# vedantsawal/Cost-and-Carbon-Aware-Kubernetes-Autoscaler

Measured on AMD Instinct MI355X. Metric: policy-evaluated cluster-steps/sec, higher is better.
Workload: dtype int32+int64+f64; 1 GPU; config2: 1e5 clusters x 1 deployment x 1440 one-minute steps, HPA + peak/off-peak, 16-type catalog; scenarios_per_gpu=100000, steps_per_rollout=1440, mode=trajectory, schedule=lane-skewed (single deployment), trace_layout=wave-tiled [wave][T][lanes] (built by the first rollout), parallelism=scenario-sharded x1

## Files before the change

cost-and-carbon-aware-kubernetes-autoscaler_amd/csrc/rollout_d1.hip:

```cpp
#include <hip/hip_runtime.h>
#include <stdint.h>

#include "../../include/ccka.h"
#include "d1_common.h"
#include "kparams.h"

#pragma clang fp contract(off)

namespace ccka {

namespace {

struct Best {
  double s;
  int k;
  int info;
  int price;
};

__device__ __forceinline__ bool better(double s2, int k2, double s, int k) {
  return s2 < s || (s2 == s && k2 < k);
}

__device__ __forceinline__ void take_if_better(Best& a, const Best& b) {
// ... 13 lines not shown
  Best o;
  const long long b = __double_as_longlong(a.s);
  const int lo = __builtin_amdgcn_readlane((int)(b & 0xffffffffLL), l);
  const int hi = __builtin_amdgcn_readlane((int)(b >> 32), l);
  o.s = __longlong_as_double(((long long)hi << 32) | (unsigned int)lo);
  o.k = __builtin_amdgcn_readlane(a.k, l);
  o.info = __builtin_amdgcn_readlane(a.info, l);
  o.price = __builtin_amdgcn_readlane(a.price, l);
  return o;
}

}

__global__ void __launch_bounds__(256) table_kernel(TableParams q) {
  const int lane = threadIdx.x & (WAVE - 1);
  const int64_t key = ((int64_t)blockIdx.x * blockDim.x + threadIdx.x) / WAVE;
  const int64_t nkeys = (int64_t)q.R * 24 * q.NZI * 3 * q.NW;
  if (key >= nkeys) return;
  int64_t x = key;
  const int wi = (int)(x % q.NW); x /= q.NW;
  const int cmi = (int)(x % 3); x /= 3;
  const int zi = (int)(x % q.NZI); x /= q.NZI;
  const int rh = (int)x;
  const uint32_t cm = (uint32_t)cmi + 1u, zm = q.zmasks[zi];
  const double wc = q.offer ? 0.0 : q.wc1000[wi];
  const double ci = q.ci_gpwh[rh];
  const int32_t* tile = q.price + (int64_t)rh * q.K * q.Z * 2;
  int2* out = q.table + key * q.JT;
  const double INF = __builtin_inf();
  Best cs{INF, 0x7fffffff, -1, 0}, ca{INF, 0x7fffffff, -1, 0};
  int jmax = 0;
  for (int base = 0; base < q.K; base += WAVE) {
    const int pos = base + lane;
    const bool v = pos < q.K;
    const int k = v ? q.order[pos] : 0;
    const int c1 = v ? q.cap1s[pos] : 0;
    const int c1n = pos + 1 < q.K ? q.cap1s[pos + 1] : 0;
    Best bs{INF, 0x7fffffff, -1, 0}, ba{INF, 0x7fffffff, -1, 0};
    if (v) {
      const double carbon = q.types[k].p_ref_w * ci;
      for (int z = 0; z < q.Z; ++z) {
        if (!(zm >> z & 1u)) continue;
        for (int c = 0; c < 2; ++c) {
          if (!(cm & (uint32_t)capbit(c))) continue;
          const int pr = tile[(k * q.Z + z) * 2 + c];
          if (pr <= 0) continue;
          const double score = (double)pr + wc * carbon;
          const int info = k | z << 10 | c << 12;
          if (score < ba.s) { ba.s = score; ba.k = k; ba.info = info; ba.price = pr; }
          if (c == 0 && score < bs.s) { bs.s = score; bs.k = k; bs.info = info; bs.price = pr; }
        }
      }
      if (ba.info >= 0) jmax = max(jmax, c1);
    }
#pragma unroll
    for (int off = 1; off < WAVE; off <<= 1) {
      const Best os = shfl_up_best(bs, off), oa = shfl_up_best(ba, off);
      if (lane >= off) { take_if_better(bs, os); take_if_better(ba, oa); }
    }
    take_if_better(bs, cs);
    take_if_better(ba, ca);
    if (v && c1 > c1n) {
      const Best& w = (!q.offer && bs.info >= 0) ? bs : ba;
      const int info = w.info >= 0 ? (w.info | q.cap1t[w.k] << 16) : -1;
      const int hi = min(c1, q.JT - 1);
      for (int n = c1n + 1; n <= hi; ++n) out[n] = make_int2(w.price, info);
    }
    cs = readlane_best(bs, WAVE - 1);
    ca = readlane_best(ba, WAVE - 1);
  }
#pragma unroll
  for (int o = 32; o > 0; o >>= 1) jmax = max(jmax, __shfl_xor(jmax, o));
  if (lane == 0) {
    q.jtab[key / q.NW] = jmax;
    out[0] = make_int2(0, jmax);
  }
}

namespace {

__device__ __forceinline__ int opqv(int v) {
  asm volatile("" : "+v"(v));
  return v;
}
__device__ __forceinline__ D1Rule opq_rule(const D1Rule& r) {
  D1Rule o;
  o.sel = opq(r.sel);
  o.n = opq(r.n);
  o.stab_mask = opq(r.stab_mask);
  o._pad = 0;
#pragma unroll
  for (int q = 0; q < 2; ++q) {
    o.type[q] = opq(r.type[q]);
    o.value[q] = opq(r.value[q]);
    o.pmask[q] = opq(r.pmask[q]);
    o.factor[q] = opq(r.factor[q]);
  }
#pragma unroll
  for (int w = 0; w < 4; ++w) {
    o.stab16[w] = opq(r.stab16[w]);
    o.pm16[0][w] = opq(r.pm16[0][w]);
    o.pm16[1][w] = opq(r.pm16[1][w]);
  }
  return o;
}

__device__ __forceinline__ int rate_limit1(const D1Rule& R, bool up, int cur, const uint32_t* del) {
  if (R.sel == CCKA_SELECT_DISABLED) return cur;
  const bool min_sel = R.sel == CCKA_SELECT_MIN;
  long long res = (up == min_sel) ? 0x7fffffffLL : -0x80000000LL;
#pragma unroll
  for (int q = 0; q < 2; ++q) {
    if (q >= R.n) break;
    int added = 0, removed = 0;
    if (R.pmask[q]) {
      const short2v z = {0, 0};
#pragma unroll
      for (int w = 0; w < 4; ++w) {
        const short2v d = as_s2(del[w]), m = as_s2((uint32_t)R.pm16[q][w]);
        added = __builtin_amdgcn_sdot2(__builtin_elementwise_max(d, z), m, added, false);
        removed = __builtin_amdgcn_sdot2(__builtin_elementwise_max(z - d, z), m, removed, false);
      }
    }
    const long long pst = (long long)cur - added + removed;
    long long pr;
    if (R.type[q] == CCKA_HPA_PODS) pr = up ? pst + R.value[q] : pst - R.value[q];
    else if (up) pr = (int)ceil((double)pst * R.factor[q]);
    else pr = (int)((double)pst * R.factor[q]);
    res = (up == min_sel) ? min(res, pr) : max(res, pr);
  }
  return (int)res;
}

}

#define D1_STAMP(k)                                          \
  if constexpr (STAMPS) {                                    \
    __builtin_amdgcn_sched_barrier(0);                       \
    const uint64_t now_ = __builtin_amdgcn_s_memtime();      \
    __builtin_amdgcn_sched_barrier(0);                       \
    st_acc[k] += now_ - st_last;                             \
    st_last = now_;                                          \
  }

constexpr int D1_RB = 64;
constexpr int D1_K = 2;
constexpr int D1_VMN = 4;
constexpr int D1_S = 8;
constexpr int D1_BACK = CCKA_HIST;
static_assert(D1_VMN + 4 * D1_S + D1_BACK <= D1_RB && D1_RB - D1_S - D1_BACK - D1_VMN >= 2 * D1_S,
              "ring too small for the DMA lead");
constexpr int D1_RING_BYTES = D1_RB * WAVE * 4;
constexpr int D1_PRIO_HI = 3;
__device__ __forceinline__ void d1_dma_row(const int32_t* src, uint32_t lds_row) {
  unsigned keep;
  asm volatile(
      "s_mov_b32 %0, m0\n\t"
      "s_mov_b32 m0, %2\n\t"
      "s_nop 0\n\t"
      "global_load_lds_dword %1, off\n\t"
      "s_mov_b32 m0, %0"
      : "=&s"(keep)
      : "v"(src), "s"(lds_row)
      : "memory");
}
__device__ __forceinline__ void d1_wait_rows() { asm volatile("s_waitcnt vmcnt(%0)" ::"n"(D1_VMN) : "memory"); }
__device__ __forceinline__ void d1_wait_all() { asm volatile("s_waitcnt vmcnt(0)" ::: "memory"); }

__device__ __forceinline__ uint32_t xcd_block(uint32_t b, uint32_t n) {
  const uint32_t x = b & 7u, k = b >> 3, q = n >> 3, r = n & 7u;
  return x * q + min(x, r) + k;
}

template <int MAXN, int MAXP, bool STAMPS, int OCC, bool BDEF, bool DRIFT = false, int NSUB = 1, int HE = 8,
          bool G3 = false, bool KEDA = false>
__global__ void __launch_bounds__(256, OCC) rollout_d1_kernel(D1Params p) {
  static_assert(NSUB == 1 || (NSUB == 4 && BDEF), "15 s sync: lean default path");
  static_assert(!KEDA || (BDEF && NSUB == 1 && !DRIFT), "KEDA: default behavior, one decision per step");
  static_assert(HE == 8 || (HE == 4 && NSUB == 1 && BDEF), "4-record ring: default behavior, one decision per step");
  static_assert(!G3 || (DRIFT && MAXP == 2), "G3: the DRIFT instantiation, two pools");
  constexpr int HW = NSUB == 1 ? HE / 2 : 10;
  constexpr int JR = NSUB == 1 ? HE : 5;
  uint64_t st_acc[12] = {0, 0, 0, 0, 0, 0, 0, 0, 0, 0, 0, 0};
  uint64_t st_last = STAMPS ? __builtin_amdgcn_s_memtime() : 0;
  extern __shared__ __attribute__((aligned(16))) int4 s_acc[];
  for (int x = threadIdx.x; x < p.K; x += blockDim.x) {
    const long long idle = p.acc[x * 3 + 0];
    s_acc[x] = make_int4((int)(idle & 0xffffffffLL), (int)(idle >> 32), (int)p.acc[x * 3 + 1], (int)p.acc[x * 3 + 2]);
  }
  const bool ldt = p.lds_tab;
  const uint32_t tab_off = ((uint32_t)p.K * 16u + 255u) / 256u * 256u + (blockDim.x / WAVE) * (uint32_t)D1_RING_BYTES;
  const int n_pr = p.R * 24 * p.K * p.Z * 2;
  const int n_pr8 = (n_pr + 1) & ~1;
  int* const s_price = reinterpret_cast<int*>(reinterpret_cast<char*>(s_acc) + tab_off);
  double* const s_ci = reinterpret_cast<double*>(s_price + n_pr8);
  int* const s_jtab = reinterpret_cast<int*>(s_ci + p.R * 24);
  if (ldt) {
    for (int x = threadIdx.x; x < n_pr; x += blockDim.x) s_price[x] = p.price[x];
    for (int x = threadIdx.x; x < p.R * 24; x += blockDim.x) s_ci[x] = p.ci_gpwmin[x];
    for (int x = threadIdx.x; x < p.R * 24 * p.NZI * 3; x += blockDim.x) s_jtab[x] = p.jtab[x];
  }
  __syncthreads();
  const int lane = threadIdx.x & (WAVE - 1);
  const int64_t wv = (int64_t)xcd_block(blockIdx.x, gridDim.x) * (blockDim.x / WAVE) + (threadIdx.x / WAVE);
  const int64_t i = wv * p.lpw + lane;
  if (lane >= p.lpw || i >= p.N) return;

  const int r = p.region ? (int)p.region[i] : 0;
  const int target = KEDA ? 1 : (p.target ? (int)p.target[i] : p.target0);
  const int mx = KEDA ? opq(p.k_max) : (p.maxr ? (int)p.maxr[i] : p.maxr0);
  const int dwin = (!KEDA && p.down_stab) ? (int)p.down_stab[i] : p.dstab0;
  const int nd = min(NSUB == 1 ? __popc(window_mask(dwin)) : (dwin > 15 ? (dwin - 1) / 15 : 0), 2 * HW);
  const int dnmask = NSUB == 1 ? window_mask(dwin) : 0;
  const int reset_ca = p.reset_ca ? (int)p.reset_ca[i] : p.reset_ca0;
  const int pswitch = p.pswitch ? (int)p.pswitch[i] : p.pswitch0;
  const int wi = p.wci ? (int)p.wci[i] : 0;
  const uint32_t capsel = p.cap_sel ? (uint32_t)p.cap_sel[i] : (uint32_t)p.capsel0;
  const int minr = KEDA ? max(opq(p.k_min), 1) : opq(p.minr), req = opq(p.req_cpu), limit = opq(p.limit);
  const int kthr = KEDA ? opq(p.k_thr) : 1, kact = KEDA ? opq(p.k_act) : 0, kcds = KEDA ? opq(p.k_cds) : 0;
  const bool kmin0 = KEDA && opq(p.k_min) == 0;
  const float rkthr = __builtin_amdgcn_rcpf((float)kthr);
  int ulo = max(0, (int)floor(p.tol_lo * (double)target) - 2);
  while ((double)ulo / (double)target < p.tol_lo) ++ulo;
  int uhi = (int)floor(p.tol_hi * (double)target) + 2;
  while ((double)uhi / (double)target > p.tol_hi) --uhi;
  const float rtarget = __builtin_amdgcn_rcpf((float)target);

  const int NP = opq(p.NP), NZI = opq(p.NZI), NW = opq(p.NW), JT = opq(p.JT);
  const int maxn = opq(p.maxn), ablate = CCKA_ABLATE_BUILD ? opq(p.ablate) : 0, pdb_member = opq(p.pdb_member);
  const int pdb_pct = opq(p.pdb_pct), slo_util = opq(p.slo_util), delay = opq(p.delay);
  const int base_nodes = opq(p.base_nodes), base_type = opq(p.base_type);
  const int K = opq(p.K), Z = opq(p.Z), T = opq(p.T);
  const int ps = opq(p.peak_start) % 1440, pe = opq(p.peak_end) % 1440;
  const int ps_raw = opq(p.peak_start), pe_raw = opq(p.peak_end);
  const int sm0 = opq(p.start_minute) % 1440;
  const long long base_nw = opq(p.base_nw);
  const GLOBAL_AS int32_t* const price = opq_ptr(p.price);
  const GLOBAL_AS double* const ci_gpwmin = opq_ptr(p.ci_gpwmin);
  const GLOBAL_AS int2* const table = opq_ptr(p.table);
  const GLOBAL_AS int2* const table2 = opq_ptr(p.table2);
  const int drift_on = opq(p.drift_on), replace = opq(p.replace), multi = G3 ? opq(p.multi) : 0;
  const GLOBAL_AS int32_t* const jtab = opq_ptr(p.jtab);
  GLOBAL_AS int4* const traj = opq_ptr(reinterpret_cast<int4*>(p.traj));
  const D1Rule rup = [&] { if constexpr (BDEF) return d1_default_rule(true); else return opq_rule(p.up); }();
  const D1Rule rdn = [&] { if constexpr (BDEF) return d1_default_rule(false); else return opq_rule(p.dn); }();
  int budget[MAXP];
#pragma unroll
  for (int q = 0; q < MAXP; ++q) budget[q] = opq(p.budget[q]);

  int ppol[MAXP], pcas[MAXP], pzi[MAXP], pJ[MAXP];
  uint32_t pcm[MAXP], pmask[MAXP];
#pragma unroll
  for (int q = 0; q < MAXP; ++q) {
    ppol[q] = 0; pcas[q] = 0; pzi[q] = -1; pcm[q] = 0; pJ[q] = 0; pmask[q] = 0;
    if (q < NP) {
#pragma unroll
      for (int s = 0; s < 2; ++s) {
        const D1Patch& x = p.patch[q][s];
        if (x.policy) ppol[q] = x.policy;
        if (x.cas >= 0) pcas[q] = s == 1 ? (reset_ca + CCKA_STEP_SECONDS - 1) / CCKA_STEP_SECONDS : x.cas;
        if (x.zi >= 0) pzi[q] = x.zi;
        if (x.cm) pcm[q] = (uint32_t)x.cm;
      }
    }
  }

  auto cas_of = [&](uint32_t info) {
    const int m1 = -(int)(info >> 13 & 1u), m2 = -(int)(info >> 14 & 1u);
    const int lo = pcas[0] ^ ((pcas[0] ^ pcas[MAXP > 1 ? 1 : 0]) & m1);
    if constexpr (MAXP <= 2) {
      return lo;
    } else {
      const int hi = pcas[2] ^ ((pcas[2] ^ pcas[3]) & m1);
      return lo ^ ((lo ^ hi) & m2);
    }
  };
  auto casc = [](int c) { return min(c, 0xFFFF); };

  uint32_t sinfo[MAXN];
  int sready[MAXN], slc[MAXN], scas[MAXN], spods[MAXN], sprice[MAXN], scap[MAXN];
  uint32_t sdyn[MAXN];
  int salloc[MAXN];
  int sallocr[MAXN];
#pragma unroll
  for (int n = 0; n < MAXN; ++n) {
    sinfo[n] = 0; sready[n] = 0; slc[n] = 0; scas[n] = 0; spods[n] = 0; sprice[n] = 0; scap[n] = 0;
    sdyn[n] = 0; salloc[n] = 0; sallocr[n] = 0;
  }
  uint32_t used = 0, rdy = 0, cmask = 0;
  auto dyn_of = [&](int n) -> uint32_t {
    if constexpr (G3) return (uint32_t)s_acc[sinfo[n] & 1023u].z;
    else return sdyn[n];
  };
  auto alloc_of = [&](int n) -> int {
    if constexpr (G3) return s_acc[sinfo[n] & 1023u].w;
    else return salloc[n];
  };
  constexpr bool kAllocR = NSUB == 1 && !G3;
  auto alloc_ready = [&](int n) -> uint32_t {
    if constexpr (kAllocR) return (uint32_t)sallocr[n];
    else return (rdy >> n & 1u) ? (uint32_t)alloc_of(n) : 0u;
  };
  auto cas_slot = [&](int n) -> int {
    if constexpr (G3) return casc(cas_of(sinfo[n]));
    else return scas[n];
  };
  uint32_t dmask = 0, srcm = 0, repm = 0;
  auto taint = [&]() -> uint32_t { return DRIFT ? (srcm | repm) : 0u; };
  auto od_slots = [&]() {
    uint32_t m = 0;
#pragma unroll
    for (int n = MAXN - 1; n >= 0; --n) m = 2 * m + (sinfo[n] >> 12 & 1u);
    return m & used;
  };
  const uint32_t slot_mask = maxn >= 32 ? 0xFFFFFFFFu : ((1u << maxn) - 1u);

  int replicas = p.replicas0, placed = 0, rpods = 0;
  uint32_t hdn[HW], hup[4], hdel[4] = {0, 0, 0, 0};
  uint32_t dn16[HW];
#pragma unroll
  for (int w = 0; w < 4; ++w) hup[w] = 0x7FFF7FFFu;
#pragma unroll
  for (int w = 0; w < HW; ++w) {
    hdn[w] = 0x80008000u;
    dn16[w] = (2 * w < nd ? 0xFFFFu : 0u) | (2 * w + 1 < nd ? 0xFFFF0000u : 0u);
  }
  int next_ready = 0x7fffffff, nsp = 0, nod = 0;
  int kcd = kcds, q_klo = 0, q_khi = -1, kb_cur = -1;
  bool q_kcd = false;
  bool k_act_step = false;
  auto keda_band = [&](int cur) {
    if (!KEDA || cur == kb_cur) return;
    kb_cur = cur;
    if (cur <= 0) { q_klo = 0; q_khi = -1; return; }
    const double D = (double)kthr * (double)cur;
// ... 60 lines not shown
    const int rc = min(max(cur, upr), dnr);
    int lo = minr, hi = mx;
    if constexpr (BDEF) {
      hi = rc > cur ? min(hi, max(2 * cur, cur + 4)) : hi;
      lo = rc < cur ? max(lo, 0) : lo;
    } else {
      if (proposal != cur) {
        if (rc > cur) hi = min(hi, max(rate_limit1(rup, true, cur, hdel), cur));
        else if (rc < cur) lo = max(lo, min(rate_limit1(rdn, false, cur, hdel), cur));
      }
    }
    return rc < lo ? lo : (rc > hi ? hi : rc);
  };
  auto hpa_eval = [&](int L, int cur, int ready, float rbd, float rbc) -> HpaOut {
    HpaOut o;
    const bool metric = cur <= mx && cur >= minr && ready > 0 && !(cur == 0 && minr != 0);
    int util = 0, proposal = cur;
    {
      const int rcapv = ready * limit;
      const int usage = (limit > 0 && rcapv < L) ? rcapv : L;
      const int a = usage * 100;
      const int dreq = ready * req;
      const int dcur = cur * req;
      bool slow = usage < 0 || usage > 21474836;
      util = fdiv_nb(a, dreq, rbd, slow);
      int nu = 0;
      if (cur > ready) nu = fdiv_nb(a, dcur, rbc, slow);
      if (__builtin_expect(metric && slow, 0))
        util = (int)(((long long)usage * 100) / ((long long)ready * req));
      const bool unready_up = cur > ready && util > target;
      int u = util, base = ready;
      if (unready_up) { u = nu; base = cur; }
      if (__builtin_expect(metric && slow && unready_up, 0))
        u = (int)(((long long)usage * 100) / ((long long)cur * req));
      const bool keep = (u >= ulo && u <= uhi) || (unready_up && u < target);
      bool slow2 = (uint32_t)u > 0xFFFFu;
      const int x = u * base;
      const int q = fdiv_nb(x, target, rtarget, slow2);
      const bool exactm = x == q * target;
      int c = q + (exactm ? 0 : 1);
      if (__builtin_expect(metric && !keep && (exactm || slow2), 0))
        c = (int)ceil(((double)u / (double)target) * (double)base);
      const int pe2 = unready_up ? max(cur, c) : c;
      proposal = (metric && !keep) ? pe2 : cur;
    }
    o.util = util;
    o.proposal = proposal;
    o.ran = metric;
    o.hpa_path = !(cur == 0 && minr != 0);
    int desired = cur > mx ? mx : (cur < minr && o.hpa_path ? minr : cur);
    if (metric && !ablated(ablate, 8)) desired = behave(proposal, cur);
    o.desired = desired;
    return o;
  };
  auto keda_eval = [&](int L, int cur, int ts) -> HpaOut {
    HpaOut o{};
    const bool act = L > kact;
    const bool cool = !act && kmin0 && ts >= kcd;
    if (act) kcd = ts + kcds;
    k_act_step = act;
    o.util = 0;
    o.proposal = cur;
    o.ran = false;
    o.hpa_path = false;
    int desired = cur;
    if (cur == 0) {
      desired = act ? 1 : 0;
    } else if (cool) {
      desired = 0;
    } else {
      o.hpa_path = true;
      if (cur > mx) {
        desired = mx;
      } else if (cur < minr) {
        desired = minr;
      } else {
        int prop = cur;
        if (L < q_klo || L > q_khi) {
          bool slow = L < 0;
          const int q = fdiv_nb(max(L, 0), kthr, rkthr, slow);
          prop = q + (q * kthr != L ? 1 : 0);
          if (__builtin_expect(slow, 0)) prop = (int)ceil((double)L / (double)kthr);
        }
        o.proposal = prop;
        o.ran = true;
        desired = ablated(ablate, 8) ? cur : behave(prop, cur);
      }
    }
    o.desired = desired;
    return o;
  };
  auto hpa_commit = [&](const HpaOut& h, int cur) {
    const int rv = min(max(h.proposal, -D1_REC_SAT - 1), D1_REC_SAT);
    ring_push<HW>(hdn, h.ran ? rv : (int)0x8000);
    if constexpr (!BDEF) {
      ring_push(hup, h.ran ? rv : 0x7FFF);
      ring_push(hdel, (h.hpa_path && h.desired != cur) ? h.desired - cur : 0);
    }
  };
  auto upp_of = [&](int L, float rbp) {
    const int rcapv = rpods * limit;
    const int usage = max((limit > 0 && rcapv < L) ? rcapv : L, 0);
    bool slow = false;
    int upp = fdiv_nb(usage, max(rpods, 1), rbp, slow);
    if (__builtin_expect(slow, 0)) upp = usage / max(rpods, 1);
    return rpods > 0 ? upp : 0;
  };
  auto dyn_energy = [&](int upp) -> long long {
    if (__builtin_expect(upp <= 0xFFFF, 1)) {
      unsigned long long ed = 0;
#pragma unroll
      for (int n = 0; n < MAXN; ++n) {
        const uint32_t use = min((uint32_t)spods[n] * (uint32_t)upp, alloc_ready(n));
        ed += (unsigned long long)dyn_of(n) * use;
      }
      return (long long)ed;
    }
    long long e = 0;
#pragma unroll
    for (int n = 0; n < MAXN; ++n) {
      const uint64_t prod = (uint64_t)(uint32_t)spods[n] * (uint64_t)(uint32_t)upp;
      const uint32_t al = alloc_ready(n);
      const uint32_t use = prod < (uint64_t)al ? (uint32_t)prod : al;
      e += (long long)((uint64_t)dyn_of(n) * use);
    }
    return e;
  };

  int t = 0;
  int nxt = 0;
  int npb = 0;
  int tq = 0;
  bool stall = false;
  auto flush = [&](int upto) {
    const int n = upto - tq;
    cost += (burn + base_price) * (long long)n;
    e_hour += (base_nw + Isum) * (long long)n;
    if constexpr (BDEF) {
      e_hour += (long long)(Ssum * (unsigned long long)usum);
      usum = 0;
    }
    pend_min += (replicas - rpods) * n;
    nmin_spot += nsp * n;
    nmin_od += nod * n;
    tq = upto;
  };

  const int64_t wtb = [&] {
    const int64_t x = wv * p.lpw;
    const uint32_t hi = (uint32_t)__builtin_amdgcn_readfirstlane((int)(x >> 32));
    const uint32_t lo = (uint32_t)__builtin_amdgcn_readfirstlane((int)(x & 0xffffffffLL));
    return (int64_t)(((uint64_t)hi << 32) | lo);
  }();
  const int32_t* lp = p.load_w ? p.load_w + wtb * T + lane
                               : p.load + (p.trace_mod > 0 ? (p.first_id + i) % p.trace_mod : i);
  const long long lsl = opq(p.load_w ? (long long)p.lpw : (long long)p.NL);
  const uint32_t ring_off = (uint32_t)__builtin_amdgcn_readfirstlane(
      (int)(((uint32_t)p.K * 16u + 255u) / 256u * 256u + (threadIdx.x / WAVE) * (uint32_t)D1_RING_BYTES));
  const uint32_t ring_lds = (uint32_t)(uintptr_t)s_acc + ring_off;
  const int* const ring = reinterpret_cast<const int*>(reinterpret_cast<const char*>(s_acc) + ring_off);
  constexpr int rsw = WAVE, rbn = D1_RB;
  auto rrow = [&](int x) { return x & (D1_RB - 1); };
  auto ridx = [&](int r) { return r * rsw + lane; };
  auto rnext = [&](int r, int q) { return (r + q) & (D1_RB - 1); };
  int tf = 0;
  int tfr = 0;
  const int32_t* lpf = lp;
  auto tf_adv = [&]() {
    ++tf;
    ++tfr;
    if (tfr == rbn) tfr = 0;
    lpf += lsl;
  };
  {
    const int n0 = min(T, D1_VMN + 4 * D1_S);
    while (tf < n0) {
      d1_dma_row(lpf, (uint32_t)__builtin_amdgcn_readfirstlane((int)(ring_lds + (uint32_t)tfr * (uint32_t)(rsw * 4))));
      tf_adv();
    }
    d1_wait_all();
  }
  int t_rdy = tf;
  bool pf_ok = false;
  bool qadv = true;
  int Lpf[D1_S];
#pragma unroll
  for (int q = 0; q < D1_S; ++q) Lpf[q] = 0;
  const int64_t w0 = wtb;
  const int wlanes = (int)min((int64_t)p.lpw, p.N - w0);
  const __amdgpu_buffer_rsrc_t trs = __builtin_amdgcn_make_buffer_rsrc(
      traj ? (void*)(reinterpret_cast<int4*>(p.traj) + w0 * T) : (void*)p.load, 0, traj ? wlanes * T * 16 : 0,
      0x00020000);
  const int lb = lane * T * 16;

  for (int it = 0;; ++it) {
    const bool live = t < T;
    if (__ballot(live) == 0) break;
    d1_wait_rows();
    t_rdy = max(t_rdy, tf - D1_VMN);
    const uint64_t sb = __ballot(stall);
    if constexpr (STAMPS) st_acc[9] += 1;
    if (sb != 0 && (it % D1_K == D1_K - 1 || !qadv)) {
      __builtin_amdgcn_s_setprio(0);
      if constexpr (STAMPS) { st_acc[10] += 1; st_acc[11] += __popcll(sb); }
      const bool ev = stall;
      int L = 0, minute = 0, rh = 0, pd = 0, step_last_type = 0xFFFF;
      int4 rec;
      uint32_t flags = 0;
      bool g_acted = false, hchg = false, jchg = false;
      uint32_t emp_e = 0, weou_e = 0;
      HpaOut hp{};
      if (ev) {
        stall = false;
        const int tr = rrow(t);
        L = ring[ridx(tr)];
        if constexpr (BDEF) {
          const int kq = min(t - tq, wr);
          if (kq > 0) {
            const int cur16 = min(replicas, D1_REC_SAT);
            int us[JR], rv[JR];
            bool anylow = false;
#pragma unroll
            for (int j = 0; j < JR; ++j) {
              us[j] = KEDA ? ring[ridx(rnext(tr, rbn - 1 - j))] : min(ring[ridx(rnext(tr, rbn - 1 - j))], q_rcap);
              rv[j] = q_met ? cur16 : (int)0x8000;
              anylow |= (j < kq) & q_met & (us[j] < q_pge);
            }
            if (KEDA && anylow) {
#pragma unroll
              for (int j = 0; j < JR; ++j) {
                bool sl = false;
                const bool low = (j < kq) & q_met & (us[j] < q_pge);
                const int q = fdiv_nb(max(us[j], 0), kthr, rkthr, sl);
                rv[j] = low ? min(q + (q * kthr != us[j] ? 1 : 0), D1_REC_SAT) : rv[j];
              }
            } else if (anylow) {
              const int dreq = rpods * req;
              const float rbd = __builtin_amdgcn_rcpf((float)dreq);
              bool anyex = false;
#pragma unroll
              for (int j = 0; j < JR; ++j) {
                bool sl = false;
                const bool low = (j < kq) & q_met & (us[j] < q_pge);
                const int util = fdiv_nb(us[j] * 100, dreq, rbd, sl);
                const int x = (int)__umul24((uint32_t)util, (uint32_t)rpods);
                const int q = fdiv_nb(x, target, rtarget, sl);
                const bool ex = x == q * target;
                anyex |= low & ex;
                rv[j] = low ? min(q + (ex ? 0 : 1), D1_REC_SAT) : rv[j];
                us[j] = (low & ex) ? util : -1;
              }
              if (__builtin_expect(anyex, 0)) {
#pragma unroll
                for (int j = 0; j < JR; ++j)
                  if (us[j] >= 0)
                    rv[j] = min((int)ceil(((double)us[j] / (double)target) * (double)rpods), D1_REC_SAT);
              }
            }
#pragma unroll
            for (int j = JR - 1; j >= 0; --j)
              if (j < kq) {
                if constexpr (NSUB == 1) ring_push<HW>(hdn, rv[j]);
                else ring_push4<HW>(hdn, rv[j]);
              }
          }
        }
        flush(t);
        minute = (sm0 + t) % 1440;
        const int h = minute / 60;
        rh = r * 24 + h;
        if (h != hour) {
          if (hour >= 0) {
            gco2 += (double)e_hour * (ci_min * 1e-9);
            energy_nw += e_hour;
          }
          e_hour = 0;
          hour = h;
          hchg = true;
        }
      }
      D1_STAMP(2);
      if (ev) {
        if (t >= next_ready) {
          next_ready = 0x7fffffff;
#pragma unroll
          for (int n = 0; n < MAXN; ++n) {
            if ((used & ~rdy) >> n & 1u) {
              if (sready[n] <= t) {
                rdy |= 1u << n;
                rpods += spods[n];
                sallocr[n] = salloc[n];
                if ((cmask & ~taint()) >> n & 1u) Ffree += scap[n] - spods[n];
              }
              else next_ready = min(next_ready, sready[n]);
            }
          }
        }
        const bool in_win = ps_raw <= pe_raw ? (minute >= ps_raw && minute < pe_raw)
                                             : (minute >= ps_raw || minute < pe_raw);
        const bool peak = pswitch && in_win;
        const int prof = peak ? CCKA_PROFILE_PEAK : CCKA_PROFILE_OFFPEAK;
        if (peak) flags |= 1u;
        q_peak = peak;
        if (prof != profile) {
          profile = prof;
          int pold[MAXP];
#pragma unroll
          for (int q = 0; q < MAXP; ++q) pold[q] = pcas[q];
#pragma unroll
          for (int q = 0; q < MAXP; ++q) {
            if (q >= NP) break;
            const D1Patch& x = p.patch[q][prof + 1];
            if (x.policy) ppol[q] = x.policy;
            if (x.cas >= 0) pcas[q] = x.cas;
            if (x.zi >= 0) pzi[q] = x.zi;
            if (x.cm) pcm[q] = (uint32_t)x.cm;
          }
#pragma unroll
          for (int n = 0; n < MAXN; ++n)
            if (used >> n & 1u) {
              const int c = casc(cas_of(sinfo[n]));
              if constexpr (G3) {
                const int m1 = -(int)(sinfo[n] >> 13 & 1u);
                const int o = pold[0] ^ ((pold[0] ^ pold[MAXP > 1 ? 1 : 0]) & m1);
                slc[n] += c - casc(o);
              } else {
                slc[n] += c - scas[n];
              }
              scas[n] = c;
            }
          jchg = true;
          if (DRIFT && drift_on) {
            uint32_t dm = 0;
#pragma unroll
            for (int n = 0; n < MAXN; ++n) {
              const uint32_t x = sinfo[n];
              uint32_t zm = 0, cm = 0;
#pragma unroll
              for (int q = 0; q < MAXP; ++q)
                if ((int)(x >> 13 & 3u) == q) { zm = pzi[q] >= 0 ? p.zml[pzi[q]] : 0u; cm = pcm[q]; }
              const bool drifted = !(zm >> (x >> 10 & 3u) & 1u) || !(cm & capbit((int)(x >> 12 & 1u)));
              dm |= ((used >> n & 1u) && drifted ? 1u : 0u) << n;
            }
            dmask = dm;
          }
        }

      }
      D1_STAMP(3);
      if (ev) {
#pragma unroll
        for (int sub = 0; sub < NSUB; ++sub) {
          const int cur = replicas;
          if constexpr (KEDA) hp = keda_eval(L, cur, t);
          else
            hp = hpa_eval(L, cur, rpods, __builtin_amdgcn_rcpf((float)(rpods * req)),
                          __builtin_amdgcn_rcpf((float)(cur * req)));
          hpa_commit(hp, cur);
          replicas = hp.desired;
        }

        if (placed > replicas) {
          int excess = placed - replicas;
          placed = replicas;
#pragma unroll
          for (int pass = 0; pass < 2; ++pass) {
            const uint32_t m = pass == 0 ? (used & ~rdy) : rdy;
            if (!m || excess <= 0) continue;
// ... 616 lines not shown
                  ffree_now();
                  break;
                }
              }
            }
          }
          if (any_del) {
            g_acted = true;
            minscap = 0x7fffffff;
#pragma unroll
            for (int n = 0; n < MAXN; ++n) minscap = (used >> n & 1u) ? min(minscap, scap[n]) : minscap;
          }
        }

        emp_e = emp;
      }
      D1_STAMP(6);
      if (ev) {
        {
          unsigned long long sv = 0;
          float rv = 0.f;
#pragma unroll
          for (int n = 0; n < MAXN; ++n) {
            const uint32_t pr = (rdy >> n & 1u) ? (uint32_t)spods[n] : 0u;
            sv += (unsigned long long)dyn_of(n) * pr;
            rv = fmaxf(rv, (float)pr * __builtin_amdgcn_rcpf((float)alloc_of(n)));
          }
          Ssum = sv;
          Rmax = rv;
        }
        q_rbp = __builtin_amdgcn_rcpf((float)rpods);
        const int upp = upp_of(L, q_rbp);
        long long e_step = base_nw + Isum;
        if ((float)upp * Rmax < 0.9999f) e_step += (long long)(Ssum * (unsigned long long)(uint32_t)upp);
        else e_step += dyn_energy(upp);
        cost += burn + base_price;
        e_hour += e_step;
        const int pending = replicas - rpods;
        const bool slo_s = KEDA ? (k_act_step && replicas == 0) : (hp.ran && hp.util > slo_util);
        if (pending > 0 || slo_s) { slo++; flags |= 8u; }
        pend_min += pending;
        nmin_spot += nsp;
        nmin_od += nod;
        peak_nodes = max(peak_nodes, nsp + nod);
        tq = t + 1;
        rec = make_int4(replicas, pending, (nsp & 0xFFFF) | nod << 16,
                        (step_last_type & 0xFFFF) | (int)(flags << 16));

        if constexpr (BDEF) {
          constexpr int UQ = 1 << 20;
          auto umin = [](int u, uint32_t d) -> int {
            const unsigned long long a = (unsigned long long)(uint32_t)u * d;
            return a > 100ull * UQ ? UQ : min((int)(((uint32_t)a + 99u) / 100u), UQ);
          };
          const bool hpa_path = !(replicas == 0 && minr != 0);
          bool met = replicas <= mx && replicas >= minr && rpods > 0 && hpa_path;
          const int dnm = replicas > mx ? mx : (replicas < minr && hpa_path ? minr : replicas);
          const bool pend = replicas > rpods;
          q_met = met;
          q_rcap = limit > 0 ? (int)__umul24((uint32_t)rpods, (uint32_t)limit) : 0x7fffffff;
          const uint32_t dreq = (uint32_t)rpods * (uint32_t)req;
          int ulim = 0, pge = UQ, slo_thr = pend ? 0 : UQ;
          if (met) {
            int uge = ulo;
            int lim;
            if (pend) {
              lim = max(umin(target + 1, dreq), umin(uhi + 1, (uint32_t)replicas * (uint32_t)req));
            } else {
              bool sl = false;
              const int cq = fdiv_nb(target + replicas - 1, replicas, __builtin_amdgcn_rcpf((float)replicas), sl);
              int us = target - cq + 1;
              const int um = us - 1;
              if (um >= 0) {
                const int xm = um * replicas;
                const int qm = fdiv_nb(xm, target, rtarget, sl);
                if (__builtin_expect(xm == qm * target, 0) &&
                    (int)ceil(((double)um / (double)target) * (double)replicas) >= replicas)
                  us = um;
              }
              uge = min(uge, max(us, 0));
              lim = umin(uhi + 1, dreq);
            }
            pge = umin(uge, dreq);
            ulim = replicas >= mx ? UQ : lim;
            if (!pend) slo_thr = umin(max(slo_util + 1, 0), dreq);
          } else if (dnm == replicas) {
            ulim = UQ;
          }
          if constexpr (KEDA) {
            met = false;
            ulim = 0;
            pge = UQ;
            slo_thr = pend ? 0 : UQ;
            q_kcd = false;
            if (replicas == 0) {
              ulim = (int)min(max((long long)kact + 1, 0LL), (long long)UQ);
              pge = 0;
            } else if (replicas >= minr && replicas <= mx) {
              met = true;
              q_kcd = kmin0;
              keda_band(replicas);
              ulim = replicas >= mx ? UQ : (int)min((long long)q_khi + 1, (long long)UQ);
              const long long lc = (long long)(replicas - 1) * kthr + 1;
              pge = (int)max(0LL, min(min((long long)q_klo, lc), (long long)UQ));
            }
            q_met = met;
          }
          q_ulim = ulim;
          q_pge = pge;
          q_slo = slo_thr;
          q_rbp = rpods > 0 ? __builtin_amdgcn_rcpf((float)rpods) : 0.f;
          q_hbp = 0.5f * q_rbp;
          q_usat = Rmax > 0.f ? (int)fminf(0.9999f * __builtin_amdgcn_rcpf(Rmax), 1073741824.0f) - 1 : 0x7fffffff;
          q_pendv = replicas - rpods;
          q_nodes = (nsp & 0xFFFF) | nod << 16;
          q_w0 = 0xFFFF | (int)((q_peak ? 1u : 0u) << 16);
          q_w1 = q_w0 | (8 << 16);
        } else {
          q_rbd = __builtin_amdgcn_rcpf((float)(rpods * req));
          q_rbc = __builtin_amdgcn_rcpf((float)(replicas * req));
        }
        if constexpr (BDEF) {
          int hit = -0x40000000;
#pragma unroll
          for (int k = 2 * HW - 1; k >= 0; --k) {
            const int e = (int)(short)(hdn[k >> 1] >> (16 * (k & 1)));
            hit = e >= replicas ? t - k / NSUB : hit;
          }
          q_hold = replicas <= minr ? 0x3fffffff : hit + wl;
          if (!q_met) q_hold = 0x3fffffff;
        }
        {
          const int th = t + 60 - minute % 60;
          int nx = min(next_ready, th);
          if (pswitch) {
            if (t >= npb) {
              const int dps = (ps - minute + 1439) % 1440 + 1, dpe = (pe - minute + 1439) % 1440 + 1;
              npb = t + min(dps, dpe);
            }
            nx = min(nx, npb);
          }
          const uint32_t gm = rdy & (emp_e | (Ffree >= minscap ? weou_e : (weou_e & ~cmask)) |
                                     ((DRIFT && replace) ? (weou_e & od_slots() & ~emp_e & ~srcm) : 0u) |
                                     ((DRIFT && G3 && multi) ? (weou_e & ~emp_e & ~taint()) : 0u));
#pragma unroll
          for (int n = 0; n < MAXN; ++n) nx = ((gm >> n & 1u) && slc[n] > t) ? min(nx, slc[n]) : nx;
          if (g_acted || ablated(ablate, 15)) nx = t + 1;
          nxt = nx;
        }
      }
      if (ev) {
        d1_store_rec(trs, lb + t * 16, rec);
        ++t;
      }
      pf_ok = pf_ok && !ev;
      D1_STAMP(7);
    }
    __builtin_amdgcn_s_setprio(D1_PRIO_HI);
    if (tf < T) {
      if (__ballot(t < T && t < tf + D1_S - rbn + D1_BACK) == 0) {
        const int n1 = min(T, tf + D1_S);
        while (tf < n1) {
          d1_dma_row(lpf, (uint32_t)__builtin_amdgcn_readfirstlane((int)(ring_lds + (uint32_t)tfr * (uint32_t)(rsw * 4))));
          tf_adv();
        }
        if (tf == T) {
          d1_wait_all();
          t_rdy = T;
        }
      }
    }
    bool adv = false;
    if (!pf_ok) {
      const int tr = rrow(t);
#pragma unroll
      for (int q = 0; q < D1_S; ++q) Lpf[q] = ring[ridx(rnext(tr, q))];
    }

    D1_STAMP(8);
    const int tlim = min(T, t_rdy);
#pragma unroll
    for (int sub = 0; sub < D1_S; ++sub) {
    if constexpr (BDEF) {
        const int L = Lpf[sub];
        const int usage = min(L, q_rcap);
        const int cv = KEDA ? L : usage;
        const bool ge = cv >= q_pge;
        bool ok = (t < nxt) & ((uint32_t)cv < (uint32_t)q_ulim) & (ge | (t <= q_hold));
        const bool kac = KEDA && L > kact;
        if constexpr (KEDA) ok = ok & (!q_kcd | kac | (t < kcd));
        const bool can = !stall & (t < tlim);
        const bool go = ok & can;
        stall = stall | (can & !ok);
        q_hold = (go & ge) ? max(q_hold, t + wl) : q_hold;
        if constexpr (KEDA) kcd = (go & kac) ? t + kcds : kcd;
        const int upp = (int)fmaf((float)usage, q_rbp, q_hbp);
        if (__builtin_expect(go & (upp > q_usat), 0)) {
          const long long corr = dyn_energy(upp) - (long long)(Ssum * (unsigned long long)(uint32_t)upp);
          e_hour += corr;
        }
        usum += go ? (uint32_t)upp : 0u;
        const bool slo_b = usage >= q_slo;
        slo += (go & slo_b) ? 1 : 0;
        d1_store_rec(trs, go ? lb + t * 16 : D1_NOSTORE, make_int4(replicas, q_pendv, q_nodes, slo_b ? q_w1 : q_w0));
        t += go ? 1 : 0;
        adv = adv | go;
    } else
    if (t < T && !stall && t < t_rdy) {
      const int L = Lpf[sub];
      int4 rec;
      if (!(stall = t >= nxt)) {
        const HpaOut h = hpa_eval(L, replicas, rpods, q_rbd, q_rbc);
        stall = h.desired != replicas;
        if (!stall) {
          hpa_commit(h, replicas);
          const int upp = upp_of(L, q_rbp);
          if ((float)upp * Rmax < 0.9999f) e_hour += (long long)(Ssum * (unsigned long long)(uint32_t)upp);
          else e_hour += dyn_energy(upp);
          const int pending = replicas - rpods;
          const bool slo_b = pending > 0 || (h.ran && h.util > slo_util);
          slo += slo_b ? 1 : 0;
          const uint32_t flags = (q_peak ? 1u : 0u) | (slo_b ? 8u : 0u);
          rec = make_int4(replicas, pending, (nsp & 0xFFFF) | nod << 16, 0xFFFF | (int)(flags << 16));
          adv = true;
          d1_store_rec(trs, lb + t * 16, rec);
          ++t;
        }
      }
    }
    }
    qadv = __ballot(adv) != 0;
    D1_STAMP(1);
    pf_ok = t + (D1_S - 1) < t_rdy;
    {
      const int tr = rrow(t);
#pragma unroll
      for (int q = 0; q < D1_S; ++q) Lpf[q] = ring[ridx(rnext(tr, q))];
    }
    D1_STAMP(8);
  }
  d1_wait_all();
  if constexpr (STAMPS) {
    if (lane == (__ffsll((long long)__ballot(1)) - 1)) {
      for (int k = 1; k < 12; ++k) atomicAdd(&p.stamps[k], (unsigned long long)st_acc[k]);
      atomicMax(&p.stamps[0], (unsigned long long)st_acc[9]);
    }
  }
  flush(T);
  energy_nw += e_hour;
  gco2 += (double)e_hour * (ci_min * 1e-9);
  p.res.cost[i] = cost;
  p.res.energy[i] = (double)energy_nw * 1e-9;
  p.res.gco2[i] = gco2;
  p.res.slo[i] = slo;
  p.res.pend_min[i] = pend_min;
  p.res.nmin_spot[i] = nmin_spot;
  p.res.nmin_od[i] = nmin_od;
  p.res.launches[i] = launches;
  p.res.deletions[i] = deletions;
  p.res.peak_nodes[i] = peak_nodes;
  p.res.final_reps[i] = replicas;
  p.res.final_nodes[i] = __popc(used);
  p.res.last_choice[i] = last_choice;
  p.res.hash[i] = hash;
}

hipError_t launch_table(const TableParams& t, hipStream_t s) {
  const int64_t nkeys = (int64_t)t.R * 24 * t.NZI * 3 * t.NW;
  const unsigned grid = (unsigned)((nkeys * WAVE + 255) / 256);
  hipLaunchKernelGGL(table_kernel, dim3(grid), dim3(256), 0, s, t);
  return hipGetLastError();
}

hipError_t launch_rollout_d1(const D1Params& p, hipStream_t s, int32_t* plan) {
  const int B = 256;
  const int64_t waves = (p.N + p.lpw - 1) / p.lpw;
  const unsigned grid = (unsigned)((waves + B / WAVE - 1) / (B / WAVE));
  size_t lds = ((size_t)p.K * sizeof(int4) + 255) / 256 * 256 + (size_t)(B / WAVE) * D1_RING_BYTES;
  const size_t npr = (size_t)p.R * 24 * p.K * p.Z * 2;
  const size_t tabB = ((npr + 1) & ~(size_t)1) * 4 + (size_t)p.R * 24 * 8 + (size_t)p.R * 24 * p.NZI * 3 * 4;
  D1Params q = p;
  q.lds_tab = 0;
  if (lds + tabB <= 80 * 1024) {
    q.lds_tab = 1;
    lds += tabB;
  }
  auto go = [&](auto kernel) { hipLaunchKernelGGL(kernel, dim3(grid), dim3(B), lds, s, q); };
  const bool d = p.bdef != 0;
  int inst = 802;
  if (p.keda) {
    if (p.he4) go(rollout_d1_kernel<8, 2, false, 2, true, false, 1, 4, false, true>);
    else go(rollout_d1_kernel<8, 2, false, 2, true, false, 1, 8, false, true>);
  } else if (p.nsub == 4) {
    if (p.multi) go(rollout_d1_kernel<8, 2, false, 2, true, true, 4, 8, true>);
    else if (p.drift) go(rollout_d1_kernel<8, 2, false, 2, true, true, 4>);
    else go(rollout_d1_kernel<8, 2, false, 2, true, false, 4>);
  } else if (p.multi) {
    if (d) go(rollout_d1_kernel<8, 2, false, 2, true, true, 1, 8, true>);
    else go(rollout_d1_kernel<8, 2, false, 2, false, true, 1, 8, true>);
  } else if (p.drift) {
    if (d) go(rollout_d1_kernel<8, 2, false, 2, true, true>);
    else go(rollout_d1_kernel<8, 2, false, 2, false, true>);
  } else if (p.stamps) {
    if (d && p.he4) go(rollout_d1_kernel<8, 2, true, 2, true, false, 1, 4>);
    else if (d) go(rollout_d1_kernel<8, 2, true, 2, true>);
    else go(rollout_d1_kernel<8, 2, true, 2, false>);
  } else if (p.maxn <= 8 && p.NP <= 2 && p.occ == 3) {
    go(rollout_d1_kernel<8, 2, false, 3, false>);
  } else if (p.maxn <= 8 && p.NP <= 2) {
    if (d && p.he4) go(rollout_d1_kernel<8, 2, false, 2, true, false, 1, 4>);
    else if (d) go(rollout_d1_kernel<8, 2, false, 2, true>);
    else go(rollout_d1_kernel<8, 2, false, 2, false>);
  } else if (p.maxn <= 8) {
    inst = 804;
    go(rollout_d1_kernel<8, 4, false, 2, false>);
  } else if (p.NP <= 2) {
    inst = 1602;
    go(rollout_d1_kernel<16, 2, false, 1, false>);
  } else {
    inst = 1604;
    go(rollout_d1_kernel<16, 4, false, 1, false>);
  }
  if (plan) {
    plan[PLAN_GRID] = (int32_t)grid;
    plan[PLAN_LDS] = (int32_t)lds;
    plan[PLAN_D1_LDS_TAB] = q.lds_tab;
    plan[PLAN_D1_INST] = inst;
  }
  return hipGetLastError();
}

}
```

Measured before the change: 78.35 billion cluster-steps/s.

## Batch trace-ring DMA with scalar-base loads and shift the prefetch window on stalls

When the wave-tiled trace layout is present, ring refills go through global_load_lds with an SGPR base plus a per-lane VGPR offset, and eight rows are issued from one inline-asm block that steps the base and m0 in scalar registers. This removes per-row 64-bit VGPR pointer arithmetic and readfirstlane overhead. Separately, the stalled-lane slow path now takes the current load from the prefetched register window and shifts that window by one row, instead of re-reading the ring and invalidating the whole prefetch. The risks are inline asm that clobbers vcc and m0, and extra register shuffling inside the slow path.

```diff
diff --git a/cost-and-carbon-aware-kubernetes-autoscaler_amd/csrc/rollout_d1.hip b/cost-and-carbon-aware-kubernetes-autoscaler_amd/csrc/rollout_d1.hip
--- a/cost-and-carbon-aware-kubernetes-autoscaler_amd/csrc/rollout_d1.hip
+++ b/cost-and-carbon-aware-kubernetes-autoscaler_amd/csrc/rollout_d1.hip
@@ -189,6 +189,12 @@
               "ring too small for the DMA lead");
 constexpr int D1_RING_BYTES = D1_RB * WAVE * 4;
 constexpr int D1_PRIO_HI = 3;
+#ifndef D1_REFILL_S
+#define D1_REFILL_S 1
+#endif
+#ifndef D1_PF_SHIFT
+#define D1_PF_SHIFT 1
+#endif
 __device__ __forceinline__ void d1_dma_row(const int32_t* src, uint32_t lds_row) {
   unsigned keep;
   asm volatile(
@@ -201,6 +207,48 @@
       : "v"(src), "s"(lds_row)
       : "memory");
 }
+__device__ __forceinline__ void d1_dma_row_s(const int32_t* sbase, uint32_t voff, uint32_t lds_row) {
+  unsigned keep;
+  asm volatile(
+      "s_mov_b32 %0, m0\n\t"
+      "s_mov_b32 m0, %3\n\t"
+      "s_nop 0\n\t"
+      "global_load_lds_dword %1, %2\n\t"
+      "s_mov_b32 m0, %0"
+      : "=&s"(keep)
+      : "v"(voff), "s"(sbase), "s"(lds_row)
+      : "memory");
+}
+#define D1_ROW_NEXT                          \
+  "s_add_u32 vcc_lo, vcc_lo, %[st]\n\t"      \
+  "s_addc_u32 vcc_hi, vcc_hi, 0\n\t"         \
+  "s_add_u32 m0, m0, 0x100\n\t"              \
+  "s_nop 0\n\t"                              \
+  "global_load_lds_dword %[vo], vcc\n\t"
+__device__ __forceinline__ void d1_dma_rows8_s(const int32_t* sbase, uint32_t stride, uint32_t voff, uint32_t lds0,
+                                               uint32_t lds4) {
+  unsigned keep;
+  asm volatile(
+      "s_mov_b32 %[keep], m0\n\t"
+      "s_mov_b64 vcc, %[sb]\n\t"
+      "s_mov_b32 m0, %[l0]\n\t"
+      "s_nop 0\n\t"
+      "global_load_lds_dword %[vo], vcc\n\t"
+      D1_ROW_NEXT D1_ROW_NEXT D1_ROW_NEXT
+      "s_add_u32 vcc_lo, vcc_lo, %[st]\n\t"
+      "s_addc_u32 vcc_hi, vcc_hi, 0\n\t"
+      "s_mov_b32 m0, %[l4]\n\t"
+      "s_nop 0\n\t"
+      "global_load_lds_dword %[vo], vcc\n\t"
+      D1_ROW_NEXT D1_ROW_NEXT D1_ROW_NEXT
+      "s_mov_b32 m0, %[keep]"
+      : [keep] "=&s"(keep)
+      : [vo] "v"(voff), [sb] "s"(sbase), [st] "s"(stride), [l0] "s"(lds0), [l4] "s"(lds4)
+      : "memory", "vcc", "scc");
+}
+#undef D1_ROW_NEXT
+static_assert(D1_S == 8 && (D1_VMN + 4 * D1_S) % 4 == 0 && D1_RB % 4 == 0 && WAVE * 4 == 0x100,
+              "d1_dma_rows8_s: 8 rows of 256 B, refills start at a multiple of 4 rows");
 __device__ __forceinline__ void d1_wait_rows() { asm volatile("s_waitcnt vmcnt(%0)" ::"n"(D1_VMN) : "memory"); }
 __device__ __forceinline__ void d1_wait_all() { asm volatile("s_waitcnt vmcnt(0)" ::: "memory"); }
 
@@ -218,6 +266,8 @@
   static_assert(!G3 || (DRIFT && MAXP == 2), "G3: the DRIFT instantiation, two pools");
   constexpr int HW = NSUB == 1 ? HE / 2 : 10;
   constexpr int JR = NSUB == 1 ? HE : 5;
+  constexpr bool kRefillS = D1_REFILL_S && OCC != 3 && !(NSUB == 4 && !DRIFT);
+  constexpr bool kPfShift = D1_PF_SHIFT && NSUB == 1;
   uint64_t st_acc[12] = {0, 0, 0, 0, 0, 0, 0, 0, 0, 0, 0, 0};
   uint64_t st_last = STAMPS ? __builtin_amdgcn_s_memtime() : 0;
   extern __shared__ __attribute__((aligned(16))) int4 s_acc[];
@@ -584,8 +634,10 @@
     const uint32_t lo = (uint32_t)__builtin_amdgcn_readfirstlane((int)(x & 0xffffffffLL));
     return (int64_t)(((uint64_t)hi << 32) | lo);
   }();
-  const int32_t* lp = p.load_w ? p.load_w + wtb * T + lane
-                               : p.load + (p.trace_mod > 0 ? (p.first_id + i) % p.trace_mod : i);
+  const bool tiled = kRefillS && p.load_w != nullptr;
+  const int32_t* lp = tiled      ? reinterpret_cast<const int32_t*>((uintptr_t)lane * 4u)
+                      : p.load_w ? p.load_w + wtb * T + lane
+                                 : p.load + (p.trace_mod > 0 ? (p.first_id + i) % p.trace_mod : i);
   const long long lsl = opq(p.load_w ? (long long)p.lpw : (long long)p.NL);
   const uint32_t ring_off = (uint32_t)__builtin_amdgcn_readfirstlane(
       (int)(((uint32_t)p.K * 16u + 255u) / 256u * 256u + (threadIdx.x / WAVE) * (uint32_t)D1_RING_BYTES));
@@ -598,22 +650,41 @@
   int tf = 0;
   int tfr = 0;
   const int32_t* lpf = lp;
-  auto tf_adv = [&]() {
-    ++tf;
-    ++tfr;
-    if (tfr == rbn) tfr = 0;
-    lpf += lsl;
+  const int32_t* srow = p.load_w + wtb * T;
+  const uint32_t srow_b = (uint32_t)__builtin_amdgcn_readfirstlane((int)lsl * 4);
+  auto lds_row = [&](int r) {
+    return (uint32_t)__builtin_amdgcn_readfirstlane((int)(ring_lds + (uint32_t)r * (uint32_t)(rsw * 4)));
   };
-  {
-    const int n0 = min(T, D1_VMN + 4 * D1_S);
-    while (tf < n0) {
-      d1_dma_row(lpf, (uint32_t)__builtin_amdgcn_readfirstlane((int)(ring_lds + (uint32_t)tfr * (uint32_t)(rsw * 4))));
-      tf_adv();
-    }
-    d1_wait_all();
-  }
+  auto fill_rows = [&](int n1) {
+    if (tiled) {
+      if (n1 - tf == D1_S) {
+        d1_dma_rows8_s(srow, srow_b, (uint32_t)(uintptr_t)lpf, lds_row(tfr), lds_row(rnext(tfr, 4)));
+        tf += D1_S;
+        tfr = rnext(tfr, D1_S);
+        srow += D1_S * lsl;
+      } else {
+        while (tf < n1) {
+          d1_dma_row_s(srow, (uint32_t)(uintptr_t)lpf, lds_row(tfr));
+          ++tf;
+          tfr = rnext(tfr, 1);
+          srow += lsl;
+        }
+      }
+    } else {
+      while (tf < n1) {
+        d1_dma_row(lpf, lds_row(tfr));
+        ++tf;
+        tfr = rnext(tfr, 1);
+        lpf += lsl;
+      }
+    }
+  };
+  fill_rows(min(T, D1_VMN + 4 * D1_S));
+  d1_wait_all();
   int t_rdy = tf;
   bool pf_ok = false;
+  int pf_rdy = -1;
+  (void)pf_rdy;
   bool qadv = true;
   int Lpf[D1_S];
 #pragma unroll
@@ -645,7 +716,7 @@
       if (ev) {
         stall = false;
         const int tr = rrow(t);
-        L = ring[ridx(tr)];
+        L = kPfShift ? Lpf[0] : ring[ridx(tr)];
         if constexpr (BDEF) {
           const int kq = min(t - tq, wr);
           if (kq > 0) {
@@ -1568,18 +1639,20 @@
       if (ev) {
         d1_store_rec(trs, lb + t * 16, rec);
         ++t;
+        if constexpr (kPfShift) {
+#pragma unroll
+          for (int q = 0; q + 1 < D1_S; ++q) Lpf[q] = Lpf[q + 1];
+          Lpf[D1_S - 1] = ring[ridx(rrow(t + D1_S - 1))];
+          pf_ok = pf_ok && t + (D1_S - 1) < t_rdy;
+        }
       }
-      pf_ok = pf_ok && !ev;
+      if constexpr (!kPfShift) pf_ok = pf_ok && !ev;
       D1_STAMP(7);
     }
     __builtin_amdgcn_s_setprio(D1_PRIO_HI);
     if (tf < T) {
       if (__ballot(t < T && t < tf + D1_S - rbn + D1_BACK) == 0) {
-        const int n1 = min(T, tf + D1_S);
-        while (tf < n1) {
-          d1_dma_row(lpf, (uint32_t)__builtin_amdgcn_readfirstlane((int)(ring_lds + (uint32_t)tfr * (uint32_t)(rsw * 4))));
-          tf_adv();
-        }
+        fill_rows(min(T, tf + D1_S));
         if (tf == T) {
           d1_wait_all();
           t_rdy = T;
@@ -1587,7 +1660,7 @@
       }
     }
     bool adv = false;
-    if (!pf_ok) {
+    if (!pf_ok && (!kPfShift || t_rdy > pf_rdy)) {
       const int tr = rrow(t);
 #pragma unroll
       for (int q = 0; q < D1_S; ++q) Lpf[q] = ring[ridx(rnext(tr, q))];
@@ -1648,6 +1721,7 @@
     qadv = __ballot(adv) != 0;
     D1_STAMP(1);
     pf_ok = t + (D1_S - 1) < t_rdy;
+    pf_rdy = t_rdy;
     {
       const int tr = rrow(t);
 #pragma unroll
```

Result: no change. 78.27 billion cluster-steps/s (median of 2 runs) (-0.1%).
